# thethomasboyer/PhenDiff

Hardware: NVIDIA B200
Metric: images/sec, DDIM invert+regenerate 128x128 100 steps (higher is better)
Workload: dtype fp16

## Files before the change

### phendiff_b200/csrc/pd_conv_halo.cu

```cuda
#include "pd_tc_common.cuh"
#include <algorithm>
#include <cstdlib>
#include <cstring>
#include <string>

namespace pd {

struct HaloParams {
    CUtensorMap tmA, tmA2, tmS1, tmS2, tmB;
    CUtensorMap tmOut;
    int ntaps, kw, pitch_px;
    int a_bytes_main, a_bytes_sc, a_stage_bytes, SA, SB;
    int kb_main, kb_s1, kb_s2, C;
    int tilesW, tilesH;
    int off_h, off_w;
    int m_tiles, n_tiles, phases, b_rows_per_phase;
    int Ho, Wo;
    int upsample;
    int mt;
    int kb_a1;
    int sc_per_stage;
    const float2* gn_coef;
    int H, W;
    int gn_tanh;
    int tile_begin, tile_end;
    TcEpi epi;
};

struct ConvHaloPlan {
    HaloParams p;
    int dt, block_n, grid, mode, gn;
    size_t smem;
};

constexpr int HL_WT = 8, HL_HT = 16;
constexpr int HL_EPI_BYTES = 8 * 4096;

template <int BLOCK_N, int MODE> struct HaloEpiWarps { static constexpr int value = (MODE == TC_MODE_STD && BLOCK_N >= 128) ? 8 : 4; };

template <int R> __device__ __forceinline__ void setmaxnreg_inc() { asm volatile("setmaxnreg.inc.sync.aligned.u32 %0;" ::"n"(R)); }
template <int R> __device__ __forceinline__ void setmaxnreg_dec() { asm volatile("setmaxnreg.dec.sync.aligned.u32 %0;" ::"n"(R)); }

template <typename T, bool TANH> __device__ __forceinline__ uint4 gn_silu8(const uint4& raw, const float4 (&cf)[4]) {
    float v[8];
    unpack8<T>(raw, v);
    const float a[8] = {cf[0].x, cf[0].z, cf[1].x, cf[1].z, cf[2].x, cf[2].z, cf[3].x, cf[3].z};
    const float b[8] = {cf[0].y, cf[0].w, cf[1].y, cf[1].w, cf[2].y, cf[2].w, cf[3].y, cf[3].w};
#pragma unroll
    for (int i = 0; i < 8; ++i) {
        const float y = fmaf(v[i], a[i], b[i]);
        if (TANH) {
            float t;
            asm("tanh.approx.f32 %0, %1;" : "=f"(t) : "f"(y));
            v[i] = fmaf(y, t, y);
        } else {
            v[i] = silu<false>(y);
        }
    }
    uint4 o;
    o.x = pack2<T>(v[0], v[1]); o.y = pack2<T>(v[2], v[3]); o.z = pack2<T>(v[4], v[5]); o.w = pack2<T>(v[6], v[7]);
    return o;
}

__device__ __forceinline__ uint4 lds128(uint32_t addr) {
    uint4 v;
    asm volatile("ld.shared.v4.u32 {%0, %1, %2, %3}, [%4];" : "=r"(v.x), "=r"(v.y), "=r"(v.z), "=r"(v.w) : "r"(addr) : "memory");
    return v;
}
__device__ __forceinline__ void sts128(uint32_t addr, const uint4& v) {
    asm volatile("st.shared.v4.u32 [%0], {%1, %2, %3, %4};" ::"r"(addr), "r"(v.x), "r"(v.y), "r"(v.z), "r"(v.w) : "memory");
}

template <typename T, bool TANH>
__device__ __forceinline__ void gn_transform_tile(uint32_t col, int r0, int nrows, int pitch, int qstep, int rstep, int hy, int hx,
                                                  int gy0, int gx0, int H, int W, const float4 (&cf)[4]) {
#pragma unroll 1
    for (int rho = r0; rho < nrows; rho += 32) {
        const bool ok0 = (unsigned)(gy0 + hy) < (unsigned)H && (unsigned)(gx0 + hx) < (unsigned)W;
        hy += qstep; hx += rstep;
        if (hx >= pitch) { hx -= pitch; ++hy; }
        const bool in1 = rho + 16 < nrows;
        const bool ok1 = in1 && (unsigned)(gy0 + hy) < (unsigned)H && (unsigned)(gx0 + hx) < (unsigned)W;
        hy += qstep; hx += rstep;
        if (hx >= pitch) { hx -= pitch; ++hy; }
        const uint32_t q0 = col + (uint32_t)rho * 128u, q1 = q0 + 2048u;
        const uint4 v0 = lds128(q0);
        const uint4 v1 = in1 ? lds128(q1) : make_uint4(0u, 0u, 0u, 0u);
        const uint4 o0 = gn_silu8<T, TANH>(v0, cf);
        const uint4 o1 = gn_silu8<T, TANH>(v1, cf);
        if (ok0) sts128(q0, o0);
        if (ok1) sts128(q1, o1);
    }
}

template <int BLOCK_N, typename T, int MODE, int CW, int MT, bool GN>
__global__ void __launch_bounds__(GN ? HALO_THREADS_GN : HALO_THREADS, 1) conv_halo_kernel(const __grid_constant__ HaloParams p) {
    constexpr int EPI_WARPS = HaloEpiWarps<BLOCK_N, MODE>::value;
    constexpr int B_BYTES = BLOCK_N * TC_BLOCK_K * 2;
    constexpr int TMEM_COLS = (2 * MT * BLOCK_N < 32) ? 32 : 2 * MT * BLOCK_N;
    static_assert(TMEM_COLS <= 512, "accumulators exceed TMEM");
    constexpr int TILE_W = HL_WT * MT;
    extern __shared__ uint8_t smem_raw[];
    uint8_t* smem = reinterpret_cast<uint8_t*>((reinterpret_cast<uintptr_t>(smem_raw) + 1023) & ~(uintptr_t)1023);
    const int SA = p.SA, SB = p.SB;
    uint8_t* smA = smem;
    uint8_t* smB = smem + (size_t)SA * p.a_stage_bytes;
    uint8_t* smEpi = smB + (size_t)SB * B_BYTES;
    uint64_t* bars = reinterpret_cast<uint64_t*>(smEpi + (MODE == TC_MODE_STD ? HL_EPI_BYTES : 0));
    uint64_t* fullA = bars;
    uint64_t* emptyA = fullA + SA;
    uint64_t* fullB = emptyA + SA;
    uint64_t* emptyB = fullB + SB;
    uint64_t* tfull = emptyB + SB;
    uint64_t* tempty = tfull + 2;
    uint64_t* readyA = tempty + 2;
    uint32_t* tmem_slot = reinterpret_cast<uint32_t*>(readyA + 4);

    const int warp = threadIdx.x >> 5, lane = threadIdx.x & 31;

    if (warp == 0 && elect_one()) {
        prefetch_tmap(&p.tmA);
        prefetch_tmap(&p.tmB);
        if (p.kb_a1 < p.kb_main) prefetch_tmap(&p.tmA2);
        if (p.kb_s1) prefetch_tmap(&p.tmS1);
        if (p.kb_s2) prefetch_tmap(&p.tmS2);
        if (MODE == TC_MODE_STD) prefetch_tmap(&p.tmOut);
    }
    if (warp == 1 && elect_one()) {
        for (int i = 0; i < SA; ++i) { mbar_init(&fullA[i], 1); mbar_init(&emptyA[i], 1); }
        for (int i = 0; i < SB; ++i) { mbar_init(&fullB[i], 1); mbar_init(&emptyB[i], 1); }
        for (int i = 0; i < 2; ++i) { mbar_init(&tfull[i], 1); mbar_init(&tempty[i], 32 * EPI_WARPS); }
        if (GN) for (int i = 0; i < SA; ++i) mbar_init(&readyA[i], 128);
        fence_barrier_init();
    }
    if (warp == 2) {
        tmem_alloc(tmem_slot, TMEM_COLS);
        tmem_relinquish();
    }
    tc_fence_before();
    __syncthreads();
    tc_fence_after();
    const uint32_t tmem_base = *tmem_slot;

    const int total_tiles = p.tile_end;
    const int tiles_per_img = p.tilesW * p.tilesH;

    if (warp < 4) {
      if (GN) setmaxnreg_dec<96>();
      if (warp == 0) {
        if (elect_one()) {
            int sb = 0;
            uint32_t phb = 0;
            for (int tile = p.tile_begin + blockIdx.x; tile < total_tiles; tile += gridDim.x) {
                const int n_tile = tile % p.n_tiles;
                const int phase = (tile / p.n_tiles) % p.phases;
                const int brow = phase * p.b_rows_per_phase + n_tile * BLOCK_N;
                int kcol = 0;
                for (int seg = 0; seg < 3; ++seg) {
                    const int nkb = seg == 0 ? p.kb_main : (seg == 1 ? p.kb_s1 : p.kb_s2);
                    const int ntap = seg == 0 ? p.ntaps : 1;
                    const int segC = nkb * TC_BLOCK_K;
                    for (int cb = 0; cb < nkb; ++cb) {
                        for (int tap = 0; tap < ntap; ++tap) {
                            mbar_wait(&emptyB[sb], phb ^ 1);
                            mbar_arrive_expect_tx(&fullB[sb], B_BYTES);
                            tma_load_2d(&p.tmB, &fullB[sb], smB + (size_t)sb * B_BYTES, kcol + tap * segC + cb * TC_BLOCK_K, brow);
                            if (++sb == SB) { sb = 0; phb ^= 1; }
                        }
                    }
                    kcol += ntap * segC;
                }
            }
        }
      } else if (warp == 3) {
        if (elect_one()) {
            int sa = 0;
            uint32_t pha = 0;
            for (int tile = p.tile_begin + blockIdx.x; tile < total_tiles; tile += gridDim.x) {
                const int t2 = tile / p.n_tiles;
                const int phase = t2 % p.phases, m_tile = t2 / p.phases;
                const int img = m_tile / tiles_per_img, rem = m_tile - img * tiles_per_img;
                const int th = rem / p.tilesW, tw = rem - th * p.tilesW;
                const int h0 = th * HL_HT, w0 = tw * TILE_W;
                const int oh = p.off_h + (p.upsample ? (phase >> 1) : 0), ow = p.off_w + (p.upsample ? (phase & 1) : 0);
                for (int seg = 0; seg < 3; ++seg) {
                    const int nkb = seg == 0 ? p.kb_main : (seg == 1 ? p.kb_s1 : p.kb_s2);
                    const int per = seg == 0 ? 1 : p.sc_per_stage;
                    for (int cb = 0; cb < nkb; cb += per) {
                        mbar_wait(&emptyA[sa], pha ^ 1);
                        uint8_t* dstA = smA + (size_t)sa * p.a_stage_bytes;
                        if (seg == 0) {
                            mbar_arrive_expect_tx(&fullA[sa], p.a_bytes_main);
                            if (cb < p.kb_a1) tma_load_4d(&p.tmA, &fullA[sa], dstA, cb * TC_BLOCK_K, w0 + ow, h0 + oh, img);
                            else tma_load_4d(&p.tmA2, &fullA[sa], dstA, (cb - p.kb_a1) * TC_BLOCK_K, w0 + ow, h0 + oh, img);
                        } else {
                            const int nb = min(per, nkb - cb);
                            mbar_arrive_expect_tx(&fullA[sa], nb * p.a_bytes_sc);
                            for (int b = 0; b < nb; ++b)
                                tma_load_4d(seg == 1 ? &p.tmS1 : &p.tmS2, &fullA[sa], dstA + (size_t)b * p.a_bytes_sc, (cb + b) * TC_BLOCK_K, w0, h0, img);
                        }
                        if (++sa == SA) { sa = 0; pha ^= 1; }
                    }
                }
            }
        }
      } else if (warp == 1) {
        if (elect_one()) {
            constexpr uint32_t idesc = make_idesc<T, BLOCK_N>();
            constexpr uint32_t B_HI = sw128_desc_hi(1024u);
            constexpr uint32_t B_LO_STEP = (uint32_t)B_BYTES >> 4;
            const int kw = p.kw, ntaps = p.ntaps, pitch_main = p.pitch_px;
            const int nkbs[3] = {p.kb_main, p.kb_s1, p.kb_s2};
            const int sc_per_stage = p.sc_per_stage;
            const uint32_t sc_blk_lo = (uint32_t)p.a_bytes_sc >> 4;
            const uint32_t a_lo0 = (smem_u32(smA) & 0x3FFFFu) >> 4, a_lo_step = (uint32_t)p.a_stage_bytes >> 4;
            const uint32_t b_lo0 = (smem_u32(smB) & 0x3FFFFu) >> 4;
            const uint32_t bar_fullA = smem_u32(GN ? readyA : fullA), bar_emptyA = smem_u32(emptyA);
            const uint32_t bar_fullB = smem_u32(fullB), bar_emptyB = smem_u32(emptyB);
            const uint32_t bar_tfull = smem_u32(tfull), bar_tempty = smem_u32(tempty);
            int sa = 0, sb = 0;
            uint32_t pha = 0, phb = 0;
            int iter = 0;
            for (int tile = p.tile_begin + blockIdx.x; tile < total_tiles; tile += gridDim.x, ++iter) {
                const int as = iter & 1;
                const uint32_t aphase = (iter >> 1) & 1;
                mbar_wait_addr(bar_tempty + as * 8, aphase ^ 1);
                tc_fence_after();
                const uint32_t d_tmem = tmem_base + (uint32_t)(as * MT * BLOCK_N);
                uint32_t accum = 0;
#pragma unroll 1
                for (int seg = 0; seg < 3; ++seg) {
                    const int nkb = nkbs[seg];
                    const int pitch = seg == 0 ? pitch_main : TILE_W;
                    const uint32_t a_hi = sw128_desc_hi((uint32_t)pitch * 128u);
                    const int per = seg == 0 ? 1 : sc_per_stage;
                    const uint32_t tap_step = seg == 0 ? 8u : sc_blk_lo;
                    const int wrap_at = seg == 0 ? kw : (1 << 30);
                    const uint32_t row_wrap = (uint32_t)(pitch - kw) * 8u;
#pragma unroll 1
                    for (int cb = 0; cb < nkb; cb += per) {
                        const int ntap = seg == 0 ? ntaps : min(per, nkb - cb);
                        mbar_wait_addr(bar_fullA + sa * 8, pha);
                        tc_fence_after();
                        uint32_t a_lo = a_lo0 + (uint32_t)sa * a_lo_step;
                        int sx = 0;
#pragma unroll 1
                        for (int tap = 0; tap < ntap; ++tap) {
                            mbar_wait_addr(bar_fullB + sb * 8, phb);
                            tc_fence_after();
                            const uint32_t b_lo = b_lo0 + (uint32_t)sb * B_LO_STEP;
#pragma unroll
                            for (int k = 0; k < TC_BLOCK_K / 16; ++k) {
#pragma unroll
                                for (int half = 0; half < MT; ++half)
                                    umma_f16kind(d_tmem + (uint32_t)(half * BLOCK_N), desc64(a_hi, a_lo + (uint32_t)(half * HL_WT * 8 + 2 * k)),
                                                 desc64(B_HI, b_lo + (uint32_t)(2 * k)), idesc, (accum | (uint32_t)k) ? 1u : 0u);
                            }
                            accum = 1;
                            umma_commit_addr(bar_emptyB + sb * 8);
                            if (++sb == SB) { sb = 0; phb ^= 1; }
                            a_lo += tap_step;
                            if (++sx == wrap_at) { sx = 0; a_lo += row_wrap; }
                        }
                        umma_commit_addr(bar_emptyA + sa * 8);
                        if (++sa == SA) { sa = 0; pha ^= 1; }
                    }
                }
                umma_commit_addr(bar_tfull + as * 8);
            }
        }
      }
    } else if (warp < 12) {
      if (GN) setmaxnreg_inc<168>();
      if (warp < 4 + EPI_WARPS) {
        const int ew = warp - 4;
        const int q = ew & 3, slab0 = ew >> 2;
        constexpr int SLAB_STEP = EPI_WARPS / 4;
        const int row = q * 32 + lane;
        const int hh = row >> 3, ww = row & 7;
        uint8_t* buf = smEpi + ew * 4096;
        int iter = 0;
        for (int tile = p.tile_begin + blockIdx.x; tile < total_tiles; tile += gridDim.x, ++iter) {
            const int n_tile = tile % p.n_tiles;
            const int t2 = tile / p.n_tiles;
            const int phase = t2 % p.phases, m_tile = t2 / p.phases;
            const int img = m_tile / tiles_per_img, rem = m_tile - img * tiles_per_img;
            const int th = rem / p.tilesW, tw = rem - th * p.tilesW;
            const int h0 = th * HL_HT, w0 = tw * TILE_W;
            const int as = iter & 1;
            const uint32_t aphase = (iter >> 1) & 1;
            mbar_wait(&tfull[as], aphase);
            tc_fence_after();
            const uint32_t t_addr = tmem_base + ((uint32_t)(q * 32) << 16) + (uint32_t)(as * MT * BLOCK_N);
            if (MODE == TC_MODE_DDIM) {
#pragma unroll
                for (int half = 0; half < MT; ++half) {
                    const int oh = h0 + hh, ow = w0 + half * HL_WT + ww;
                    const int hw = oh * p.Wo + ow;
                    uint32_t r[16];
                    tmem_ld_32x32b_x16(t_addr + (uint32_t)(half * BLOCK_N), r);
                    tmem_ld_wait();
                    if (half == MT - 1) {
                        tc_fence_before();
                        mbar_arrive(&tempty[as]);
                    }
                    tc_epilogue_ddim(p.epi, r, img, hw);
                }
            } else {
                constexpr int SLABS = BLOCK_N >= 64 ? BLOCK_N / 64 : 1, ITEMS = MT * SLABS;
#pragma unroll 1
                for (int item = slab0; item < ITEMS; item += SLAB_STEP) {
                    const int half = item / SLABS, slab = item - half * SLABS;
                    const int wh = w0 + half * HL_WT;
                    int oh = h0 + hh, ow = wh + ww;
                    if (p.upsample) { oh = 2 * oh + (phase >> 1); ow = 2 * ow + (phase & 1); }
                    const size_t pix = (size_t)img * p.Ho * p.Wo + (size_t)oh * p.Wo + ow;
                    const int col0 = n_tile * BLOCK_N + slab * 64;
                    const uint32_t t_item = t_addr + (uint32_t)(half * BLOCK_N + slab * 64);
                    uint32_t r0[32], r1[32];
                    tmem_ld_32x32b_x32(t_item, r0);
                    tmem_ld_32x32b_x32(t_item + 32u, r1);
                    uint4 res[8];
                    const bool has_res = p.epi.residual != nullptr;
                    if (has_res) {
                        const T* rbase = reinterpret_cast<const T*>(p.epi.residual) + col0 + (lane & 7) * 8;
#pragma unroll
                        for (int k = 0; k < 8; ++k) {
                            const int i = (lane >> 3) + 4 * k;
                            const size_t rp = (size_t)img * p.Ho * p.Wo + (size_t)(h0 + 4 * q + (i >> 3)) * p.Wo + (wh + (i & 7));
                            res[k] = __ldg(reinterpret_cast<const uint4*>(rbase + rp * p.epi.Cout));
                        }
                    }
                    if (lane == 0) bulk_wait_read<0>();
                    __syncwarp();
                    if (has_res) {
#pragma unroll
                        for (int k = 0; k < 8; ++k) {
                            const int i = (lane >> 3) + 4 * k;
                            *reinterpret_cast<uint4*>(buf + i * 128 + (((lane & 7) ^ (i & 7)) << 4)) = res[k];
                        }
                        __syncwarp();
#pragma unroll
                        for (int c = 0; c < 8; ++c) res[c] = *reinterpret_cast<const uint4*>(buf + lane * 128 + ((c ^ (lane & 7)) << 4));
                        __syncwarp();
                    }
                    tmem_ld_wait();
                    if (item + SLAB_STEP >= ITEMS) {
                        tc_fence_before();
                        mbar_arrive(&tempty[as]);
                    }
                    tc_epilogue_chunk32<T, true, CW>(p.epi, r0, col0, pix, img, lane, buf + lane * 128, 0, res, has_res);
                    tc_epilogue_chunk32<T, true, CW>(p.epi, r1, col0 + 32, pix, img, lane, buf + lane * 128, 4, res + 4, has_res);
                    fence_proxy_async();
                    __syncwarp();
                    if (lane == 0) {
                        if (p.upsample) tma_store_5d(&p.tmOut, buf, col0, phase & 1, wh, phase >> 1, img * (p.Ho >> 1) + h0 + 4 * q);
                        else tma_store_4d(&p.tmOut, buf, col0, wh, h0 + 4 * q, img);
                        bulk_commit();
                    }
                }
            }
        }
        if (MODE == TC_MODE_STD && lane == 0) bulk_wait_read<0>();
      }
    } else if (GN) {
        setmaxnreg_dec<80>();
        const int t = threadIdx.x - 384;
        const int j = t & 7, r0 = t >> 3;
        const int lc = j ^ (r0 & 7);
        const int pitch = p.pitch_px;
        const int nrows = pitch * (HL_HT + 2);
        const int qstep = 16 / pitch, rstep = 16 - qstep * pitch;
        int hy0 = 0, hx0 = r0;
        while (hx0 >= pitch) { hx0 -= pitch; ++hy0; }
        int sa = 0;
        uint32_t pha = 0;
        asm volatile("griddepcontrol.wait;" ::: "memory");
        for (int tile = p.tile_begin + blockIdx.x; tile < total_tiles; tile += gridDim.x) {
            const int t2 = tile / p.n_tiles;
            const int m_tile = t2 / p.phases;
            const int img = m_tile / tiles_per_img, rem = m_tile - img * tiles_per_img;
            const int th = rem / p.tilesW, tw = rem - th * p.tilesW;
            const int gy0 = th * HL_HT + p.off_h, gx0 = tw * TILE_W + p.off_w;
            const float2* crow = p.gn_coef + (size_t)img * p.C + lc * 8;
            for (int seg = 0; seg < 3; ++seg) {
                const int nkb = seg == 0 ? p.kb_main : (seg == 1 ? p.kb_s1 : p.kb_s2);
                const int per = seg == 0 ? 1 : p.sc_per_stage;
                for (int cb = 0; cb < nkb; cb += per) {
                    float4 cf[4];
                    if (seg == 0) {
                        const float4* cp = reinterpret_cast<const float4*>(crow + cb * TC_BLOCK_K);
#pragma unroll
                        for (int i = 0; i < 4; ++i) cf[i] = __ldg(cp + i);
                        if (p.gn_tanh) {
#pragma unroll
                            for (int i = 0; i < 4; ++i) { cf[i].x *= 0.5f; cf[i].y *= 0.5f; cf[i].z *= 0.5f; cf[i].w *= 0.5f; }
                        }
                    }
                    mbar_wait(&fullA[sa], pha);
                    if (seg == 0) {
                        const uint32_t col = smem_u32(smA + (size_t)sa * p.a_stage_bytes + j * 16);
                        if (p.gn_tanh) gn_transform_tile<T, true>(col, r0, nrows, pitch, qstep, rstep, hy0, hx0, gy0, gx0, p.H, p.W, cf);
                        else gn_transform_tile<T, false>(col, r0, nrows, pitch, qstep, rstep, hy0, hx0, gy0, gx0, p.H, p.W, cf);
                        fence_proxy_async();
                    }
                    mbar_arrive(&readyA[sa]);
                    if (++sa == SA) { sa = 0; pha ^= 1; }
                }
            }
        }
    }
    tc_fence_before();
    __syncthreads();
    if (warp == 2) {
        tc_fence_after();
        tmem_dealloc(tmem_base, TMEM_COLS);
    }
}

static int halo_block_n(const ConvTcDesc& d) {
    if (d.mode == TC_MODE_DDIM) return d.Cout <= 16 ? 16 : 0;
    static const int lin128 = [] { const char* e = getenv("PHENDIFF_B200_HALO_LIN128"); return e ? atoi(e) : 1; }();
    if (lin128 && d.ksize == 1 && !d.upsample && d.Cout % 128 == 0 && d.W % (2 * HL_WT) == 0) return 128;
    if (d.Cout % 256 == 0) return 256;
    if (d.Cout % 128 == 0) return 128;
    if (d.Cout % 64 == 0) return 64;
    return 0;
}

bool conv_halo_supported(const ConvTcDesc& d, std::string* why) {
    auto no = [&](const char* m) { if (why) *why = m; return false; };
    if (const char* off = getenv("PHENDIFF_B200_HALO")) if (off[0] == '0') return no("halo kernel disabled by PHENDIFF_B200_HALO=0");
    if (d.dt != DT_BF16 && d.dt != DT_F16) return no("tcgen05 path takes bf16 or fp16 activations");
    if (d.C % 64 != 0 || d.C2 % 64 != 0 || d.Csc1 % 64 != 0 || d.Csc2 % 64 != 0) return no("channel counts must be multiples of 64");
    if (d.C2 < 0 || d.C2 >= d.C + (d.C == 0)) return no("second main-segment source must leave channels for the first");
    if (d.gn_coef && (d.ksize != 3 || d.upsample)) return no("fused GroupNorm: plain 3x3 convolution only");
    if (d.gn_coef && d.mode == TC_MODE_STD && halo_block_n(d) < 128) return no("fused GroupNorm: Cout must be a multiple of 128");
    if (halo_block_n(d) == 0) return no("Cout must be a multiple of 64 (or <= 16 for the conv_out mode)");
    if (d.stride != 1) return no("halo kernel takes stride-1 convolutions");
    if (!(d.ksize == 1 || d.ksize == 3)) return no("kernel size must be 1 or 3");
    if (d.pad != d.ksize / 2) return no("convolution must be 'same'");
    if (d.upsample) {
        if (d.ksize != 3 || d.Ho != 2 * d.H || d.Wo != 2 * d.W || d.Csc1 || d.Csc2) return no("upsample mode: 3x3, 2x output, no shortcut");
    } else if (d.Ho != d.H || d.Wo != d.W) return no("output extent must equal the input extent");
    if (d.W % HL_WT != 0 || d.H % HL_HT != 0) return no("extent must tile into 16x8-pixel boxes");
    if (d.mode == TC_MODE_DDIM && (d.upsample || d.Csc1 || d.residual || d.addvec || d.stats_out)) return no("conv_out mode takes a plain 3x3 conv");
    if (d.stats_out && d.stats_cw != 4 && d.stats_cw != 2) return no("fused statistics need a chunk width of 4 or 2");
    return true;
}

int conv_halo_plan_create(const ConvTcDesc& d, ConvHaloPlan** out) {
    std::string why;
    PD_REQUIRE(conv_halo_supported(d, &why), ("conv_halo: unsupported shape: " + why).c_str());
    ConvHaloPlan* pl = new ConvHaloPlan();
    HaloParams& p = pl->p;
    memset(&p, 0, sizeof(p));
    pl->dt = d.dt; pl->mode = d.mode; pl->block_n = halo_block_n(d); pl->gn = d.gn_coef != nullptr;
    p.gn_coef = d.gn_coef; p.H = d.H; p.W = d.W;
    {
        const char* e = getenv("PHENDIFF_B200_GN_SILU");
        p.gn_tanh = e ? (std::string(e) == "tanh") : 1;
    }
    const int kh = d.upsample ? 2 : d.ksize, kw = kh;
    p.ntaps = kh * kw; p.kw = kw;
    const char* pk = getenv("PHENDIFF_B200_HALO_PITCH");
    const bool pow2 = pk && std::string(pk) == "pow2";
    int mt = 1;
    if (pl->block_n <= 128 && d.W % (2 * HL_WT) == 0 && !pow2) mt = 2;
    if (const char* e = getenv("PHENDIFF_B200_HALO_MT")) mt = (atoi(e) == 2 && mt == 2) ? 2 : 1;
    p.mt = mt;
    const int tile_w = HL_WT * mt;
    p.pitch_px = (kw == 1) ? tile_w : (pow2 ? 16 : tile_w + kw - 1);
    const int rows = HL_HT + kh - 1;
    p.a_bytes_main = 128 * p.pitch_px * rows;
    p.a_bytes_sc = 128 * tile_w * HL_HT;
    p.sc_per_stage = 1;
    p.a_stage_bytes = ((std::max(p.a_bytes_main, p.a_bytes_sc) + 1023) / 1024) * 1024;
    p.C = d.C; p.kb_main = d.C / 64; p.kb_s1 = d.Csc1 / 64; p.kb_s2 = d.Csc2 / 64;
    p.kb_a1 = (d.C - d.C2) / 64;
    p.tilesW = d.W / tile_w; p.tilesH = d.H / HL_HT;
    p.off_h = p.off_w = d.upsample ? -1 : -d.pad;
    p.m_tiles = d.N * p.tilesW * p.tilesH;
    p.phases = d.upsample ? 4 : 1;
    const int cout_rows = d.mode == TC_MODE_DDIM ? 16 : d.Cout;
    p.b_rows_per_phase = cout_rows;
    p.n_tiles = cout_rows / pl->block_n;
    p.Ho = d.Ho; p.Wo = d.Wo; p.upsample = d.upsample;
    TcEpi& e = p.epi;
    e.bias = d.bias; e.addvec = d.addvec; e.addvec_row = d.addvec_row; e.addvec_stride = d.addvec_stride;
    e.residual = d.residual; e.out_scale = d.out_scale; e.out = d.out; e.stats = d.stats_out; e.stats_cw = d.stats_cw;
    e.Cout = d.Cout; e.c_valid = d.Cout; e.plane = d.Ho * d.Wo;
    const int b_bytes = pl->block_n * 128;
    const int epi_bytes = d.mode == TC_MODE_STD ? HL_EPI_BYTES : 0;
    const int budget = 227 * 1024 - 1024 - 512 - epi_bytes;
    p.SA = (pl->block_n >= 256 || mt == 2) ? 2 : 3;
    if (pl->block_n == 16) p.SA = 4;
    if (d.ksize == 1 && d.mode == TC_MODE_STD && d.C >= 128) {
        static const int lin_sa = [] { const char* e = getenv("PHENDIFF_B200_HALO_LIN_SA"); return e ? atoi(e) : 4; }();
        p.SA = std::min(4, std::max(2, lin_sa));
    }
    if (d.gn_coef) {
        if (mt == 2 && pl->block_n != 16) p.SA = 3;
        if (const char* e = getenv("PHENDIFF_B200_HALO_GN_SA")) p.SA = std::min(4, std::max(2, atoi(e)));
    }
    if (d.Csc1 >= 128 || d.Csc2 >= 128) {
        static const int sc2 = [] { const char* e = getenv("PHENDIFF_B200_HALO_SC2"); return e ? atoi(e) : 1; }();
        const int stage2 = ((std::max(p.a_bytes_main, 2 * p.a_bytes_sc) + 1023) / 1024) * 1024;
        if (sc2 && stage2 <= 48 * 1024 && (budget - p.SA * stage2) / b_bytes >= 4) { p.sc_per_stage = 2; p.a_stage_bytes = stage2; }
    }
    p.SB = std::min(16, (budget - p.SA * p.a_stage_bytes) / b_bytes);
    if (p.SB < 2) { delete pl; set_error("conv_halo: shared memory budget too small"); return 1; }
    pl->smem = (size_t)p.SA * p.a_stage_bytes + (size_t)p.SB * b_bytes + epi_bytes + 1024 + 512;
    const uint64_t C = d.C, H = d.H, W = d.W, N = d.N;
    int rc;
    {
        const void* srcs[2] = {d.x, d.x2};
        const uint64_t cs[2] = {C - (uint64_t)d.C2, (uint64_t)d.C2};
        CUtensorMap* tms[2] = {&p.tmA, &p.tmA2};
        for (int i = 0; i < 2; ++i) {
            if (!cs[i]) continue;
            uint64_t dims[4] = {cs[i], W, H, N};
            uint64_t st[3] = {cs[i] * 2, W * cs[i] * 2, H * W * cs[i] * 2};
            uint32_t box[4] = {64, (uint32_t)p.pitch_px, (uint32_t)rows, 1};
            if ((rc = tc_encode_map(tms[i], d.dt, srcs[i], 4, dims, st, box))) { delete pl; return rc; }
        }
    }
    const void* scs[2] = {d.sc1, d.sc2};
    const int cscs[2] = {d.Csc1, d.Csc2};
    CUtensorMap* tms[2] = {&p.tmS1, &p.tmS2};
    for (int i = 0; i < 2; ++i) {
        if (!cscs[i]) continue;
        uint64_t Cs = cscs[i];
        uint64_t dims[4] = {Cs, W, H, N};
        uint64_t st[3] = {Cs * 2, W * Cs * 2, H * W * Cs * 2};
        uint32_t box[4] = {64, (uint32_t)tile_w, HL_HT, 1};
        if ((rc = tc_encode_map(tms[i], d.dt, scs[i], 4, dims, st, box))) { delete pl; return rc; }
    }
    {
        const uint64_t Ktot = (uint64_t)(p.ntaps * p.kb_main + p.kb_s1 + p.kb_s2) * 64;
        uint64_t dims[2] = {Ktot, (uint64_t)cout_rows * p.phases};
        uint64_t st[1] = {Ktot * 2};
        uint32_t box[2] = {64, (uint32_t)pl->block_n};
        if ((rc = tc_encode_map(&p.tmB, d.dt, d.wmat, 2, dims, st, box))) { delete pl; return rc; }
    }
    if (d.mode == TC_MODE_STD) {
        const uint64_t Co = d.Cout;
        if (!d.upsample) {
            uint64_t dims[4] = {Co, (uint64_t)d.Wo, (uint64_t)d.Ho, N};
            uint64_t st[3] = {Co * 2, d.Wo * Co * 2, (uint64_t)d.Ho * d.Wo * Co * 2};
            uint32_t box[4] = {64, HL_WT, 4, 1};
            rc = tc_encode_map(&p.tmOut, d.dt, d.out, 4, dims, st, box);
        } else {
            uint64_t dims[5] = {Co, 2, W, 2, N * H};
            uint64_t st[4] = {Co * 2, 2 * Co * 2, 2 * W * Co * 2, 4 * W * Co * 2};
            uint32_t box[5] = {64, 1, HL_WT, 1, 4};
            rc = tc_encode_map(&p.tmOut, d.dt, d.out, 5, dims, st, box);
        }
        if (rc) { delete pl; return rc; }
    }
    p.tile_begin = 0; p.tile_end = p.m_tiles * p.phases * p.n_tiles;
    pl->grid = std::min(p.tile_end, tc_num_sms());
    *out = pl;
    return 0;
}

void conv_halo_plan_destroy(ConvHaloPlan* p) { delete p; }

template <int BLOCK_N, typename T, int MODE, int CW, int MT, bool GN>
static int launch_halo(const ConvHaloPlan* pl, const HaloParams& p, cudaStream_t s) {
    static size_t attr_smem_dev[PD_MAX_DEVICES] = {0};
    size_t& attr_smem = attr_smem_dev[pd_cur_dev()];
    if (pl->smem > attr_smem) {
        PD_CHECK_CUDA(cudaFuncSetAttribute(conv_halo_kernel<BLOCK_N, T, MODE, CW, MT, GN>, cudaFuncAttributeMaxDynamicSharedMemorySize,
                                           (int)pl->smem));
        attr_smem = pl->smem;
    }
    if (GN) {
        static const int pdl = [] { const char* e = getenv("PHENDIFF_B200_PDL"); return e ? atoi(e) : 1; }();
        cudaLaunchConfig_t cfg = {};
        cfg.gridDim = dim3(std::min(pl->grid, p.tile_end - p.tile_begin)); cfg.blockDim = dim3(HALO_THREADS_GN); cfg.dynamicSmemBytes = pl->smem; cfg.stream = s;
        cudaLaunchAttribute at[1];
        at[0].id = cudaLaunchAttributeProgrammaticStreamSerialization;
        at[0].val.programmaticStreamSerializationAllowed = 1;
        cfg.attrs = at; cfg.numAttrs = pdl ? 1 : 0;
        PD_CHECK_CUDA(cudaLaunchKernelEx(&cfg, conv_halo_kernel<BLOCK_N, T, MODE, CW, MT, GN>, p));
        return 0;
    }
    conv_halo_kernel<BLOCK_N, T, MODE, CW, MT, GN><<<std::min(pl->grid, p.tile_end - p.tile_begin), HALO_THREADS, pl->smem, s>>>(p);
    PD_CHECK_CUDA(cudaGetLastError());
    return 0;
}

template <int BLOCK_N, typename T, bool GN>
static int launch_halo_std(const ConvHaloPlan* pl, cudaStream_t s) {
    const bool cw2 = pl->p.epi.stats != nullptr && pl->p.epi.stats_cw == 2;
    if (BLOCK_N <= 128 && pl->p.mt == 2)
        return cw2 ? launch_halo<(BLOCK_N <= 128 ? BLOCK_N : 128), T, TC_MODE_STD, 2, 2, GN>(pl, pl->p, s)
                   : launch_halo<(BLOCK_N <= 128 ? BLOCK_N : 128), T, TC_MODE_STD, 4, 2, GN>(pl, pl->p, s);
    return cw2 ? launch_halo<BLOCK_N, T, TC_MODE_STD, 2, 1, GN>(pl, pl->p, s) : launch_halo<BLOCK_N, T, TC_MODE_STD, 4, 1, GN>(pl, pl->p, s);
}

int conv_halo_launch(const ConvHaloPlan* pl, cudaStream_t s, const ConvTcLaunch* extra) {
    if (pl->mode == TC_MODE_DDIM) {
        PD_REQUIRE(extra != nullptr, "conv_out plan needs per-launch outputs");
        HaloParams p = pl->p;
        p.epi.model_out = extra->model_out;
        p.epi.x_t = extra->x_t;
        p.epi.cfg = extra->cfg;
        if (extra->img_count > 0) {
            const int per_img = p.tilesW * p.tilesH;
            PD_REQUIRE(p.n_tiles == 1 && p.phases == 1 && extra->img_begin >= 0 && (extra->img_begin + extra->img_count) * per_img <= p.tile_end,
                       "conv_out image range outside the plan");
            p.tile_begin = extra->img_begin * per_img;
            p.tile_end = (extra->img_begin + extra->img_count) * per_img;
            p.epi.img_off = extra->img_begin;
        }
        if (extra->x_t) {
            PD_REQUIRE(extra->step != nullptr, "x_t update needs step coefficients");
            PD_REQUIRE(extra->step->sigma == 0.f, "fused conv_out update requires eta == 0");
            p.epi.step = *extra->step;
        }
        PD_DISPATCH_HALF(pl->dt, T, {
            if (pl->gn) return p.mt == 2 ? launch_halo<16, T, TC_MODE_DDIM, 4, 2, true>(pl, p, s) : launch_halo<16, T, TC_MODE_DDIM, 4, 1, true>(pl, p, s);
            return p.mt == 2 ? launch_halo<16, T, TC_MODE_DDIM, 4, 2, false>(pl, p, s) : launch_halo<16, T, TC_MODE_DDIM, 4, 1, false>(pl, p, s);
        });
    }
    if (pl->gn) {
        PD_DISPATCH_HALF(pl->dt, T, {
            switch (pl->block_n) {
                case 256: return launch_halo_std<256, T, true>(pl, s);
                case 128: return launch_halo_std<128, T, true>(pl, s);
            }
        });
        set_error("conv_halo: fused GroupNorm needs a 128- or 256-channel output tile");
        return 1;
    }
    PD_DISPATCH_HALF(pl->dt, T, {
        switch (pl->block_n) {
            case 256: return launch_halo_std<256, T, false>(pl, s);
            case 128: return launch_halo_std<128, T, false>(pl, s);
            case 64: return launch_halo_std<64, T, false>(pl, s);
        }
    });
    set_error("conv_halo: bad block_n");
    return 1;
}

}
```

Baseline: 15.25.

## Add swapped-operand halo conv tile with 256-pixel UMMA and direct epilogue

Adds a swapped mode for the halo convolution, used when output channels fit 128-channel tiles. Weights become the M operand and a taller 8x32 pixel tile becomes the N=256 operand, so one UMMA per k-step replaces several. A new epilogue reads the transposed TMEM accumulators and writes outputs directly from registers, with pair shuffles, residual adds and GroupNorm statistics, instead of staging through shared memory and storing with TMA. This cuts instruction issue and frees epilogue smem, at the cost of uncoalesced global stores and larger halo tiles that may reduce grid parallelism.

```diff
diff --git a/phendiff_b200/csrc/pd_conv_halo.cu b/phendiff_b200/csrc/pd_conv_halo.cu
--- a/phendiff_b200/csrc/pd_conv_halo.cu
+++ b/phendiff_b200/csrc/pd_conv_halo.cu
@@ -34,6 +34,7 @@
 };
 
 constexpr int HL_WT = 8, HL_HT = 16;
+constexpr int HL_SWAP = 0, HL_HT_SWAP = 32;
 constexpr int HL_EPI_BYTES = 8 * 4096;
 
 template <int BLOCK_N, int MODE> struct HaloEpiWarps { static constexpr int value = (MODE == TC_MODE_STD && BLOCK_N >= 128) ? 8 : 4; };
@@ -93,20 +94,81 @@
     }
 }
 
+template <typename T> __device__ __forceinline__ float2 unpack2(uint32_t w);
+template <> __device__ __forceinline__ float2 unpack2<bf16>(uint32_t w) { return make_float2(__uint_as_float(w << 16), __uint_as_float(w & 0xffff0000u)); }
+template <> __device__ __forceinline__ float2 unpack2<f16>(uint32_t w) { return __half22float2(*reinterpret_cast<const __half2*>(&w)); }
+
+template <typename T, int CW>
+__device__ __forceinline__ void halo_epilogue_swapped(const TcEpi& e, uint32_t t_addr, uint64_t* tempty_bar, int c, int img, size_t pix0,
+                                                      int Wo, int lane) {
+    const float bc = e.bias ? __ldg(e.bias + c) : 0.f;
+    const float ac = e.addvec ? __ldg(e.addvec + (size_t)(e.addvec_row ? e.addvec_row[img] : img) * e.addvec_stride + c) : 0.f;
+    const int odd = lane & 1;
+    const int cpair = c - odd;
+    const uint32_t* res = reinterpret_cast<const uint32_t*>(e.residual);
+    uint32_t* out = reinterpret_cast<uint32_t*>(e.out);
+    float s1 = 0.f, s2 = 0.f;
+#pragma unroll 1
+    for (int chunk = 0; chunk < 4; ++chunk) {
+        uint32_t r[32];
+        tmem_ld_32x32b_x32(t_addr + (uint32_t)(chunk * 32), r);
+        const size_t pixc = pix0 + (size_t)(4 * chunk) * Wo + odd;
+        uint32_t rw[16];
+        if (res) {
+#pragma unroll
+            for (int k = 0; k < 16; ++k) rw[k] = __ldg(res + (((pixc + (size_t)(k >> 2) * Wo + (2 * k & 7)) * e.Cout + cpair) >> 1));
+        }
+        tmem_ld_wait();
+        if (chunk == 3) {
+            tc_fence_before();
+            mbar_arrive(tempty_bar);
+        }
+#pragma unroll
+        for (int k = 0; k < 16; ++k) {
+            const float a0 = __uint_as_float(r[2 * k]) + bc + ac, a1 = __uint_as_float(r[2 * k + 1]) + bc + ac;
+            const float keep = odd ? a1 : a0;
+            const float recv = __shfl_xor_sync(0xffffffffu, odd ? a0 : a1, 1);
+            float lo = odd ? recv : keep, hi = odd ? keep : recv;
+            if (res) {
+                const float2 rv = unpack2<T>(rw[k]);
+                lo += rv.x; hi += rv.y;
+            }
+            if (e.out_scale != 1.0f) { lo *= e.out_scale; hi *= e.out_scale; }
+            s1 += lo + hi;
+            s2 += lo * lo + hi * hi;
+            out[((pixc + (size_t)(k >> 2) * Wo + (2 * k & 7)) * e.Cout + cpair) >> 1] = pack2<T>(lo, hi);
+        }
+    }
+    if (e.stats) {
+        s1 += __shfl_xor_sync(0xffffffffu, s1, 1);
+        s2 += __shfl_xor_sync(0xffffffffu, s2, 1);
+        if (CW == 4) {
+            s1 += __shfl_xor_sync(0xffffffffu, s1, 2);
+            s2 += __shfl_xor_sync(0xffffffffu, s2, 2);
+        }
+        if ((lane & (CW - 1)) < 2)
+            atomicAdd(e.stats + ((size_t)img * (e.Cout / CW) + c / CW) * 2 + (lane & 1), (double)((lane & 1) ? s2 : s1));
+    }
+}
+
 template <int BLOCK_N, typename T, int MODE, int CW, int MT, bool GN>
 __global__ void __launch_bounds__(GN ? HALO_THREADS_GN : HALO_THREADS, 1) conv_halo_kernel(const __grid_constant__ HaloParams p) {
+    constexpr bool SWAP = MT == HL_SWAP;
+    static_assert(!SWAP || (BLOCK_N == 128 && MODE == TC_MODE_STD), "swapped tile: 128 output channels, STD epilogue");
     constexpr int EPI_WARPS = HaloEpiWarps<BLOCK_N, MODE>::value;
     constexpr int B_BYTES = BLOCK_N * TC_BLOCK_K * 2;
-    constexpr int TMEM_COLS = (2 * MT * BLOCK_N < 32) ? 32 : 2 * MT * BLOCK_N;
+    constexpr int ACC_COLS = SWAP ? 2 * BLOCK_N : MT * BLOCK_N;
+    constexpr int TMEM_COLS = (2 * ACC_COLS < 32) ? 32 : 2 * ACC_COLS;
     static_assert(TMEM_COLS <= 512, "accumulators exceed TMEM");
-    constexpr int TILE_W = HL_WT * MT;
+    constexpr int TILE_W = SWAP ? HL_WT : HL_WT * MT;
+    constexpr int TILE_H = SWAP ? HL_HT_SWAP : HL_HT;
     extern __shared__ uint8_t smem_raw[];
     uint8_t* smem = reinterpret_cast<uint8_t*>((reinterpret_cast<uintptr_t>(smem_raw) + 1023) & ~(uintptr_t)1023);
     const int SA = p.SA, SB = p.SB;
     uint8_t* smA = smem;
     uint8_t* smB = smem + (size_t)SA * p.a_stage_bytes;
     uint8_t* smEpi = smB + (size_t)SB * B_BYTES;
-    uint64_t* bars = reinterpret_cast<uint64_t*>(smEpi + (MODE == TC_MODE_STD ? HL_EPI_BYTES : 0));
+    uint64_t* bars = reinterpret_cast<uint64_t*>(smEpi + (MODE == TC_MODE_STD && !SWAP ? HL_EPI_BYTES : 0));
     uint64_t* fullA = bars;
     uint64_t* emptyA = fullA + SA;
     uint64_t* fullB = emptyA + SA;
@@ -124,7 +186,7 @@
         if (p.kb_a1 < p.kb_main) prefetch_tmap(&p.tmA2);
         if (p.kb_s1) prefetch_tmap(&p.tmS1);
         if (p.kb_s2) prefetch_tmap(&p.tmS2);
-        if (MODE == TC_MODE_STD) prefetch_tmap(&p.tmOut);
+        if (MODE == TC_MODE_STD && !SWAP) prefetch_tmap(&p.tmOut);
     }
     if (warp == 1 && elect_one()) {
         for (int i = 0; i < SA; ++i) { mbar_init(&fullA[i], 1); mbar_init(&emptyA[i], 1); }
@@ -181,7 +243,7 @@
                 const int phase = t2 % p.phases, m_tile = t2 / p.phases;
                 const int img = m_tile / tiles_per_img, rem = m_tile - img * tiles_per_img;
                 const int th = rem / p.tilesW, tw = rem - th * p.tilesW;
-                const int h0 = th * HL_HT, w0 = tw * TILE_W;
+                const int h0 = th * TILE_H, w0 = tw * TILE_W;
                 const int oh = p.off_h + (p.upsample ? (phase >> 1) : 0), ow = p.off_w + (p.upsample ? (phase & 1) : 0);
                 for (int seg = 0; seg < 3; ++seg) {
                     const int nkb = seg == 0 ? p.kb_main : (seg == 1 ? p.kb_s1 : p.kb_s2);
@@ -206,7 +268,7 @@
         }
       } else if (warp == 1) {
         if (elect_one()) {
-            constexpr uint32_t idesc = make_idesc<T, BLOCK_N>();
+            constexpr uint32_t idesc = make_idesc<T, SWAP ? 2 * BLOCK_N : BLOCK_N>();
             constexpr uint32_t B_HI = sw128_desc_hi(1024u);
             constexpr uint32_t B_LO_STEP = (uint32_t)B_BYTES >> 4;
             const int kw = p.kw, ntaps = p.ntaps, pitch_main = p.pitch_px;
@@ -226,7 +288,7 @@
                 const uint32_t aphase = (iter >> 1) & 1;
                 mbar_wait_addr(bar_tempty + as * 8, aphase ^ 1);
                 tc_fence_after();
-                const uint32_t d_tmem = tmem_base + (uint32_t)(as * MT * BLOCK_N);
+                const uint32_t d_tmem = tmem_base + (uint32_t)(as * ACC_COLS);
                 uint32_t accum = 0;
 #pragma unroll 1
                 for (int seg = 0; seg < 3; ++seg) {
@@ -251,10 +313,15 @@
                             const uint32_t b_lo = b_lo0 + (uint32_t)sb * B_LO_STEP;
 #pragma unroll
                             for (int k = 0; k < TC_BLOCK_K / 16; ++k) {
-#pragma unroll
-                                for (int half = 0; half < MT; ++half)
-                                    umma_f16kind(d_tmem + (uint32_t)(half * BLOCK_N), desc64(a_hi, a_lo + (uint32_t)(half * HL_WT * 8 + 2 * k)),
-                                                 desc64(B_HI, b_lo + (uint32_t)(2 * k)), idesc, (accum | (uint32_t)k) ? 1u : 0u);
+                                if constexpr (SWAP) {
+                                    umma_f16kind(d_tmem, desc64(B_HI, b_lo + (uint32_t)(2 * k)), desc64(a_hi, a_lo + (uint32_t)(2 * k)), idesc,
+                                                 (accum | (uint32_t)k) ? 1u : 0u);
+                                } else {
+#pragma unroll
+                                    for (int half = 0; half < MT; ++half)
+                                        umma_f16kind(d_tmem + (uint32_t)(half * BLOCK_N), desc64(a_hi, a_lo + (uint32_t)(half * HL_WT * 8 + 2 * k)),
+                                                     desc64(B_HI, b_lo + (uint32_t)(2 * k)), idesc, (accum | (uint32_t)k) ? 1u : 0u);
+                                }
                             }
                             accum = 1;
                             umma_commit_addr(bar_emptyB + sb * 8);
@@ -286,13 +353,16 @@
             const int phase = t2 % p.phases, m_tile = t2 / p.phases;
             const int img = m_tile / tiles_per_img, rem = m_tile - img * tiles_per_img;
             const int th = rem / p.tilesW, tw = rem - th * p.tilesW;
-            const int h0 = th * HL_HT, w0 = tw * TILE_W;
+            const int h0 = th * TILE_H, w0 = tw * TILE_W;
             const int as = iter & 1;
             const uint32_t aphase = (iter >> 1) & 1;
             mbar_wait(&tfull[as], aphase);
             tc_fence_after();
-            const uint32_t t_addr = tmem_base + ((uint32_t)(q * 32) << 16) + (uint32_t)(as * MT * BLOCK_N);
-            if (MODE == TC_MODE_DDIM) {
+            const uint32_t t_addr = tmem_base + ((uint32_t)(q * 32) << 16) + (uint32_t)(as * ACC_COLS);
+            if (SWAP) {
+                halo_epilogue_swapped<T, CW>(p.epi, t_addr + (uint32_t)(slab0 * 128), &tempty[as], n_tile * BLOCK_N + q * 32 + lane, img,
+                                             (size_t)img * p.Ho * p.Wo + (size_t)(h0 + slab0 * 16) * p.Wo + w0, p.Wo, lane);
+            } else if (MODE == TC_MODE_DDIM) {
 #pragma unroll
                 for (int half = 0; half < MT; ++half) {
                     const int oh = h0 + hh, ow = w0 + half * HL_WT + ww;
@@ -361,7 +431,7 @@
                 }
             }
         }
-        if (MODE == TC_MODE_STD && lane == 0) bulk_wait_read<0>();
+        if (MODE == TC_MODE_STD && !SWAP && lane == 0) bulk_wait_read<0>();
       }
     } else if (GN) {
         setmaxnreg_dec<80>();
@@ -369,7 +439,7 @@
         const int j = t & 7, r0 = t >> 3;
         const int lc = j ^ (r0 & 7);
         const int pitch = p.pitch_px;
-        const int nrows = pitch * (HL_HT + 2);
+        const int nrows = pitch * (TILE_H + 2);
         const int qstep = 16 / pitch, rstep = 16 - qstep * pitch;
         int hy0 = 0, hx0 = r0;
         while (hx0 >= pitch) { hx0 -= pitch; ++hy0; }
@@ -381,7 +451,7 @@
             const int m_tile = t2 / p.phases;
             const int img = m_tile / tiles_per_img, rem = m_tile - img * tiles_per_img;
             const int th = rem / p.tilesW, tw = rem - th * p.tilesW;
-            const int gy0 = th * HL_HT + p.off_h, gx0 = tw * TILE_W + p.off_w;
+            const int gy0 = th * TILE_H + p.off_h, gx0 = tw * TILE_W + p.off_w;
             const float2* crow = p.gn_coef + (size_t)img * p.C + lc * 8;
             for (int seg = 0; seg < 3; ++seg) {
                 const int nkb = seg == 0 ? p.kb_main : (seg == 1 ? p.kb_s1 : p.kb_s2);
@@ -468,17 +538,21 @@
     int mt = 1;
     if (pl->block_n <= 128 && d.W % (2 * HL_WT) == 0 && !pow2) mt = 2;
     if (const char* e = getenv("PHENDIFF_B200_HALO_MT")) mt = (atoi(e) == 2 && mt == 2) ? 2 : 1;
+    const char* se = getenv("PHENDIFF_B200_HALO_SWAP");
+    const bool swap = !(se && se[0] == '0') && d.mode == TC_MODE_STD && (d.Cout == 128 || (d.ksize == 1 && d.Cout % 128 == 0 && d.Cout <= 512)) &&
+                      !d.upsample && !pow2 && d.H % HL_HT_SWAP == 0 && d.W % HL_WT == 0;
+    if (swap) { mt = HL_SWAP; pl->block_n = 128; }
     p.mt = mt;
-    const int tile_w = HL_WT * mt;
+    const int tile_w = swap ? HL_WT : HL_WT * mt, tile_h = swap ? HL_HT_SWAP : HL_HT;
     p.pitch_px = (kw == 1) ? tile_w : (pow2 ? 16 : tile_w + kw - 1);
-    const int rows = HL_HT + kh - 1;
+    const int rows = tile_h + kh - 1;
     p.a_bytes_main = 128 * p.pitch_px * rows;
-    p.a_bytes_sc = 128 * tile_w * HL_HT;
+    p.a_bytes_sc = 128 * tile_w * tile_h;
     p.sc_per_stage = 1;
     p.a_stage_bytes = ((std::max(p.a_bytes_main, p.a_bytes_sc) + 1023) / 1024) * 1024;
     p.C = d.C; p.kb_main = d.C / 64; p.kb_s1 = d.Csc1 / 64; p.kb_s2 = d.Csc2 / 64;
     p.kb_a1 = (d.C - d.C2) / 64;
-    p.tilesW = d.W / tile_w; p.tilesH = d.H / HL_HT;
+    p.tilesW = d.W / tile_w; p.tilesH = d.H / tile_h;
     p.off_h = p.off_w = d.upsample ? -1 : -d.pad;
     p.m_tiles = d.N * p.tilesW * p.tilesH;
     p.phases = d.upsample ? 4 : 1;
@@ -491,7 +565,7 @@
     e.residual = d.residual; e.out_scale = d.out_scale; e.out = d.out; e.stats = d.stats_out; e.stats_cw = d.stats_cw;
     e.Cout = d.Cout; e.c_valid = d.Cout; e.plane = d.Ho * d.Wo;
     const int b_bytes = pl->block_n * 128;
-    const int epi_bytes = d.mode == TC_MODE_STD ? HL_EPI_BYTES : 0;
+    const int epi_bytes = d.mode == TC_MODE_STD && !swap ? HL_EPI_BYTES : 0;
     const int budget = 227 * 1024 - 1024 - 512 - epi_bytes;
     p.SA = (pl->block_n >= 256 || mt == 2) ? 2 : 3;
     if (pl->block_n == 16) p.SA = 4;
@@ -533,7 +607,7 @@
         uint64_t Cs = cscs[i];
         uint64_t dims[4] = {Cs, W, H, N};
         uint64_t st[3] = {Cs * 2, W * Cs * 2, H * W * Cs * 2};
-        uint32_t box[4] = {64, (uint32_t)tile_w, HL_HT, 1};
+        uint32_t box[4] = {64, (uint32_t)tile_w, (uint32_t)tile_h, 1};
         if ((rc = tc_encode_map(tms[i], d.dt, scs[i], 4, dims, st, box))) { delete pl; return rc; }
     }
     {
@@ -594,6 +668,8 @@
 template <int BLOCK_N, typename T, bool GN>
 static int launch_halo_std(const ConvHaloPlan* pl, cudaStream_t s) {
     const bool cw2 = pl->p.epi.stats != nullptr && pl->p.epi.stats_cw == 2;
+    if (BLOCK_N == 128 && pl->p.mt == HL_SWAP)
+        return cw2 ? launch_halo<128, T, TC_MODE_STD, 2, HL_SWAP, GN>(pl, pl->p, s) : launch_halo<128, T, TC_MODE_STD, 4, HL_SWAP, GN>(pl, pl->p, s);
     if (BLOCK_N <= 128 && pl->p.mt == 2)
         return cw2 ? launch_halo<(BLOCK_N <= 128 ? BLOCK_N : 128), T, TC_MODE_STD, 2, 2, GN>(pl, pl->p, s)
                    : launch_halo<(BLOCK_N <= 128 ? BLOCK_N : 128), T, TC_MODE_STD, 4, 2, GN>(pl, pl->p, s);
```

After: 15.64, median of 6. 2.5% higher.
